# olibridge01/TeXOCR

Hardware: AMD Instinct MI355X
Metric: images/sec (OCRModel.generate, greedy, max_len=256, 224x672 px) (higher is better)
Workload: dtype bf16; 1 GPU; BASELINE configs[1]: config.yml dims (256-d/8h/4L enc + 4L dec, patch 16, PatchEmbedding C=3), batch 64/GPU, 224x672, greedy max_len=256; global_batch=64, parallelism=dp1 (images sharded, single process, no collective)

## Files before the change

### texocr_amd/csrc/common.h

```cpp
#pragma once
#include <hip/hip_runtime.h>
#include <hip/hip_bf16.h>
#include <stdint.h>

namespace txo {

typedef float f32x4 __attribute__((ext_vector_type(4)));
typedef __bf16 bf16x8 __attribute__((ext_vector_type(8)));
typedef uint32_t u32x4 __attribute__((ext_vector_type(4)));

constexpr int WAVE = 64;
constexpr float LN_EPS = 1e-5f;
constexpr float ATTN_SCALE = 0.125f;
constexpr int DH = 64;

template <typename T> struct Elem;
template <> struct Elem<float> {
    static constexpr int PER16 = 4;
    static constexpr int KCHUNK = 16;
    __device__ static inline float from_f32(float v) { return v; }
    __device__ static inline float to_f32(float v) { return v; }
};
template <> struct Elem<__hip_bfloat16> {
    static constexpr int PER16 = 8;
// ... 115 lines not shown
__device__ inline float ln_apply(float y, float mean, float rstd, float g, float b) { const float t = y - mean; return t * rstd * g + b; }

__device__ inline float gelu_erf(float x) { return 0.5f * x * (1.0f + erff(x * 0.70710678118654752440f)); }
__device__ inline float sigmoidf(float x) { return 1.0f / (1.0f + expf(-x)); }

__device__ inline float gelu_fast(float x) {
    const float z = x * 0.70710678118654752440f, a = fabsf(z);
    const float t = __builtin_amdgcn_rcpf(fmaf(0.3275911f, a, 1.0f));
    float p = fmaf(1.061405429f, t, -1.453152027f);
    p = fmaf(p, t, 1.421413741f); p = fmaf(p, t, -0.284496736f); p = fmaf(p, t, 0.254829592f);
    const float e = __builtin_amdgcn_exp2f(-a * a * 1.4426950408889634f);
    const float erf_abs = fmaf(-p * t, e, 1.0f);
    return 0.5f * x * (1.0f + copysignf(erf_abs, z));
}
__device__ inline float sigmoid_fast(float x) { return __builtin_amdgcn_rcpf(1.0f + __builtin_amdgcn_exp2f(-x * 1.4426950408889634f)); }
template <bool FAST> __device__ inline float gelu_sel(float x) { if constexpr (FAST) return gelu_fast(x); else return gelu_erf(x); }
template <bool FAST> __device__ inline float sigmoid_sel(float x) { if constexpr (FAST) return sigmoid_fast(x); else return sigmoidf(x); }

__device__ inline int swz128(int row, int piece) { return row * 128 + ((piece ^ (row & 7)) << 4); }

struct FastDiv {
    uint32_t d, m, l;
    FastDiv() : d(1), m(1), l(0) {}
    explicit FastDiv(uint32_t div) : d(div) {
        l = 0;
        while ((1u << l) < div) ++l;
        m = (uint32_t)((((uint64_t)1 << 32) * (((uint64_t)1 << l) - div)) / div + 1);
    }
    __host__ __device__ inline uint32_t div(uint32_t n) const {
#if defined(__HIP_DEVICE_COMPILE__)
        return (uint32_t)(((uint64_t)__umulhi(n, m) + n) >> l);
#else
        return (uint32_t)(((((uint64_t)n * m) >> 32) + n) >> l);
#endif
    }
    __host__ __device__ inline void divmod(uint32_t n, uint32_t& q, uint32_t& r) const { q = div(n); r = n - q * d; }
};

__device__ inline u32x4 ld16(const void* p) { return *reinterpret_cast<const u32x4*>(p); }
__device__ inline u32x4 ld16_stream(const void* p) { return __builtin_nontemporal_load(reinterpret_cast<const u32x4*>(p)); }
__device__ inline void st16(void* p, const u32x4& v) { *reinterpret_cast<u32x4*>(p) = v; }
#ifndef TXO_EXP_MALL
#define TXO_EXP_MALL 0
#endif
__device__ inline u32x4 ld16_once(const void* p) { if constexpr (TXO_EXP_MALL) return ld16_stream(p); else return ld16(p); }

__device__ inline float4 lds_ld_f4(unsigned addr) {
#if defined(__HIP_DEVICE_COMPILE__)
    return *reinterpret_cast<const __attribute__((address_space(3))) float4*>((uintptr_t)addr);
#else
    (void)addr; return float4{};
#endif
}

}
```

### texocr_amd/csrc/dec_gemm.h

```cpp
#pragma once
#include "common.h"

namespace txo {

enum { PRO_NONE = 0, PRO_EMBED = 1, PRO_LN2 = 2, PRO_LNF = 3 };
enum { EPI_QKV = 0, EPI_Q = 1, EPI_GLU_RES = 2, EPI_GEGLU = 3, EPI_BIAS_RES = 4, EPI_LOGITS = 5, EPI_STORE_T = 6 };

template <bool COH> __device__ inline float ldc_f32(const float* p) {
    if constexpr (!COH) return *p;
    else return __uint_as_float(__hip_atomic_load(reinterpret_cast<const unsigned*>(p), __ATOMIC_RELAXED, __HIP_MEMORY_SCOPE_AGENT));
}
template <bool COH> __device__ inline long long ldc_i64(const int64_t* p) {
    if constexpr (!COH) return *p;
    else return (long long)__hip_atomic_load(reinterpret_cast<const unsigned long long*>(p), __ATOMIC_RELAXED, __HIP_MEMORY_SCOPE_AGENT);
}
template <bool COH> __device__ inline u32x4 ldc16(const void* p) {
    if constexpr (!COH) return ld16(p);
    else {
        const unsigned long long* q = reinterpret_cast<const unsigned long long*>(p);
        const unsigned long long lo = __hip_atomic_load(q, __ATOMIC_RELAXED, __HIP_MEMORY_SCOPE_AGENT);
        const unsigned long long hi = __hip_atomic_load(q + 1, __ATOMIC_RELAXED, __HIP_MEMORY_SCOPE_AGENT);
        u32x4 r; r.x = (unsigned)lo; r.y = (unsigned)(lo >> 32); r.z = (unsigned)hi; r.w = (unsigned)(hi >> 32);
        return r;
    }
}
template <bool COH, typename E> __device__ inline u32x4 ldc16_at(const E* base, size_t off) {
    if constexpr (!COH) return ld16(base + off);
    else {
        const __amdgpu_buffer_rsrc_t r = __builtin_amdgcn_make_buffer_rsrc(const_cast<E*>(base), 0, 0x7fffffff, 0x00020000);
        return __builtin_amdgcn_raw_buffer_load_b128(r, (int)(off * sizeof(E)), 0, 16);
    }
}
template <bool COH> __device__ inline float4 ldc_f4_at(const float* base, size_t off) {
    const u32x4 r = ldc16_at<COH>(base, off);
    return make_float4(__uint_as_float(r.x), __uint_as_float(r.y), __uint_as_float(r.z), __uint_as_float(r.w));
}
template <bool COH> __device__ inline float4 ldc_f4(const float* p) {
    const u32x4 r = ldc16<COH>(p);
    return make_float4(__uint_as_float(r.x), __uint_as_float(r.y), __uint_as_float(r.z), __uint_as_float(r.w));
}
struct NoWait { __device__ inline void operator()() const {} };

constexpr int wfrag_regs(int KW, int BN) { return KW * (BN == 32 ? 2 : 1); }
constexpr int WBUF_REGS = 8;
struct WBuf { u32x4 r[WBUF_REGS]; };

template <typename T> struct DecGemmArgs {
    int rows, N, K;
    const T* W;
    int w_tiled;
    const float* bias;
    const T* A;
    const float* y;
    float* x_out;
    const float* gamma; const float* beta;
    unsigned ln_lds;
    const int64_t* tok; const float* tok_emb; const float* pos_emb;
    const int* t_ptr;
    int t_host;
    float* q_out;
    T* k_cache; T* v_cache;
    int inner, heads, tmax;
    const float* resid; float* y_out; int D;
    T* h_out; int F;
    T* z_cache;
    float* logits;
    unsigned long long* stamps;
    int a_tiled;
};

constexpr int DG_BM = 16, DG_BN = 32, DG_GROUP = 8;

template <int NVMAX, bool FAST>
__device__ inline void ln16(float4 (&v)[NVMAX], int nv, const float4 (&g)[NVMAX], const float4 (&b)[NVMAX], float inv_d) {
    float s = 0.f;
#pragma unroll
    for (int i = 0; i < NVMAX; ++i) if (i < nv) s += (v[i].x + v[i].y) + (v[i].z + v[i].w);
    const float mean = row16_sum(s) * inv_d;
    float q = 0.f;
#pragma unroll
    for (int i = 0; i < NVMAX; ++i) if (i < nv) {
        v[i].x -= mean; v[i].y -= mean; v[i].z -= mean; v[i].w -= mean;
        q += (v[i].x * v[i].x + v[i].y * v[i].y) + (v[i].z * v[i].z + v[i].w * v[i].w);
    }
    const float rstd = rsqrt_sel<FAST>(row16_sum(q) * inv_d + LN_EPS);
#pragma unroll
    for (int i = 0; i < NVMAX; ++i) if (i < nv) {
        v[i].x = v[i].x * rstd * g[i].x + b[i].x; v[i].y = v[i].y * rstd * g[i].y + b[i].y;
        v[i].z = v[i].z * rstd * g[i].z + b[i].z; v[i].w = v[i].w * rstd * g[i].w + b[i].w;
    }
}

template <typename T>
__device__ inline int a_off(int r, int k, int row_bytes, int pmask) {
    const int piece = (k * (int)sizeof(T)) >> 4;
    return r * row_bytes + ((piece ^ (r & pmask)) << 4) + ((k * (int)sizeof(T)) & 15);
}

template <typename T, int KW, int BN>
__device__ __forceinline__ void dec_gemm_prefetch(WBuf& f, const T* W, int N, int bx, int tid, bool real, int tiled = 0) {
    static_assert(KW > 0, "compile-time K only");
    constexpr int PER16 = Elem<T>::PER16, KCH = Elem<T>::KCHUNK, K = KW * 4 * KCH;
    static_assert(wfrag_regs(KW, BN) <= WBUF_REGS, "prefetch buffer too small");
    const int lane = tid & 63, wave = __builtin_amdgcn_readfirstlane(tid >> 6), lr = lane & 15, lg = lane >> 4;
    const int n0 = real ? bx * BN : 0;
    const T* w0 = W + (size_t)min(n0 + lr, N - 1) * K + lg * PER16;
    const T* w1 = W + (size_t)min(n0 + 16 + lr, N - 1) * K + lg * PER16;
    int wstep = KCH;
    if (tiled) {
// ... 59 lines not shown
            const int kc = wave + 4 * (g0 + c);
            fw0[c] = ld16(w0 + (size_t)kc * wstep); if constexpr (TWO) fw1[c] = ld16(w1 + (size_t)kc * wstep);
        }
    };
    auto load_a_global = [&](int g0) {
        const int m = min(m0 + lr, rows - 1);
        const bool at = !COH && a.a_tiled;
        const size_t abase = at ? ((size_t)(m >> 4) * nch * 16 + (m & 15)) * KCH : (size_t)m * K;
        const int astep = at ? 16 * KCH : KCH;
#pragma unroll
        for (int c = 0; c < GROUP; ++c) if (g0 + c < my_nch)
            fa[c] = ldc16_at<COH>(a.A, abase + (size_t)(wave + 4 * (g0 + c)) * astep + lg * PER16);
    };
    if constexpr (HASPRE) {
        static_assert(FIXED && wfrag_regs(KW, BN) <= WBUF_REGS, "prefetched fragments need a compile-time K that fits the buffer");
#pragma unroll
        for (int c = 0; c < GROUP; ++c) { fw0[c] = pre.r[c]; if constexpr (TWO) fw1[c] = pre.r[(KW + c) % WBUF_REGS]; }
    } else {
        load_w(0);
    }
    [[maybe_unused]] float4 lng[NVMAX], lnb[NVMAX];
    if constexpr (PRO != PRO_NONE) {
        const int sub = tid & 15, nv = FIXED ? NVMAX : K >> 6;
#pragma unroll
        for (int i = 0; i < NVMAX; ++i) if (i < nv) {
            if (COH && a.ln_lds) {
                lng[i] = lds_ld_f4(a.ln_lds + (i * 64 + sub * 4) * 4);
                lnb[i] = lds_ld_f4(a.ln_lds + (K + i * 64 + sub * 4) * 4);
            } else {
                lng[i] = *reinterpret_cast<const float4*>(a.gamma + i * 64 + sub * 4);
                lnb[i] = *reinterpret_cast<const float4*>(a.beta + i * 64 + sub * 4);
            }
        }
    }
    wait_prev();
    if constexpr (EPI == EPI_GLU_RES) {
        e_res0 = ldc_f32<COH>(a.resid + (size_t)emc * a.D + (n0 >> 1) + (lr & 7));
        if constexpr (TWO) e_res1 = ldc_f32<COH>(a.resid + (size_t)emc * a.D + (n0 >> 1) + 8 + (lr & 7));
    } else if constexpr (EPI == EPI_BIAS_RES) {
        e_res0 = ldc_f32<COH>(a.resid + (size_t)emc * a.D + na); e_res1 = ldc_f32<COH>(a.resid + (size_t)emc * a.D + nb);
    }
    int t = 0;
    if constexpr (PRO == PRO_EMBED || EPI == EPI_QKV || (EPI == EPI_STORE_T && PRO != PRO_NONE)) t = a.t_host >= 0 ? a.t_host : *a.t_ptr;
    if constexpr (PRO == PRO_NONE) load_a_global(0);
    __builtin_amdgcn_sched_barrier(0);

    if constexpr (PRO != PRO_NONE) {
        const int sub = tid & 15, r = tid >> 4, nv = FIXED ? NVMAX : K >> 6;
        const float inv_d = 1.0f / K;
        const int m = min(m0 + r, rows - 1);
        float4 v[NVMAX];
        float4 (&g)[NVMAX] = lng; float4 (&b)[NVMAX] = lnb;
        if constexpr (PRO == PRO_EMBED) {
            const float* te = a.tok_emb + (size_t)ldc_i64<COH>(a.tok + m) * K;
            const float* pe = a.pos_emb + (size_t)t * K;
#pragma unroll
            for (int i = 0; i < NVMAX; ++i) if (i < nv) {
                const float4 p = *reinterpret_cast<const float4*>(te + i * 64 + sub * 4);
                const float4 q = *reinterpret_cast<const float4*>(pe + i * 64 + sub * 4);
                v[i] = make_float4(p.x + q.x, p.y + q.y, p.z + q.z, p.w + q.w);
            }
        } else {
#pragma unroll
            for (int i = 0; i < NVMAX; ++i) if (i < nv)
                v[i] = ldc_f4_at<COH>(a.y, (size_t)m * K + i * 64 + sub * 4);
        }
        if constexpr (PRO == PRO_LN2) ln16<NVMAX, sizeof(T) == 2>(v, nv, g, b, inv_d);
        if constexpr (PRO == PRO_EMBED || PRO == PRO_LN2) {
            if (bx == 0 && valid && m0 + r < rows) {
#pragma unroll
                for (int i = 0; i < NVMAX; ++i) if (i < nv)
                    *reinterpret_cast<float4*>(a.x_out + (size_t)m * K + i * 64 + sub * 4) = v[i];
            }
        }
        ln16<NVMAX, sizeof(T) == 2>(v, nv, g, b, inv_d);
        [[maybe_unused]] T* zrow = nullptr;
        if constexpr (EPI == EPI_STORE_T) { if (a.z_cache && bx == 0 && valid && m0 + r < rows) zrow = a.z_cache + ((size_t)m * a.tmax + t) * K; }
#pragma unroll
        for (int i = 0; i < NVMAX; ++i) if (i < nv) {
            unsigned char* dst = smem + a_off<T>(r, i * 64 + sub * 4, row_bytes, pmask);
            if constexpr (sizeof(T) == 4) {
                *reinterpret_cast<float4*>(dst) = v[i];
                if constexpr (EPI == EPI_STORE_T) { if (zrow) *reinterpret_cast<float4*>(zrow + i * 64 + sub * 4) = v[i]; }
            } else {
                union { bf16 h[4]; uint2 u; } c;
                c.h[0] = __float2bfloat16(v[i].x); c.h[1] = __float2bfloat16(v[i].y);
                c.h[2] = __float2bfloat16(v[i].z); c.h[3] = __float2bfloat16(v[i].w);
                *reinterpret_cast<uint2*>(dst) = c.u;
                if constexpr (EPI == EPI_STORE_T) { if (zrow) *reinterpret_cast<uint2*>(zrow + i * 64 + sub * 4) = c.u; }
            }
        }
        __syncthreads();
    }

    f32x4 acc0 = {0.f, 0.f, 0.f, 0.f}, acc1 = {0.f, 0.f, 0.f, 0.f};
    for (int g0 = 0; g0 < my_nch; g0 += GROUP) {
        if (g0 > 0) { load_w(g0); if constexpr (PRO == PRO_NONE) load_a_global(g0); }
        if constexpr (PRO != PRO_NONE) {
#pragma unroll
            for (int c = 0; c < GROUP; ++c) if (g0 + c < my_nch)
                fa[c] = ld16(smem + a_off<T>(lr, (wave + 4 * (g0 + c)) * KCH + lg * PER16, row_bytes, pmask));
        }
#pragma unroll
        for (int c = 0; c < GROUP; ++c) if (g0 + c < my_nch) { mma16<T>(acc0, fa[c], fw0[c]); if constexpr (TWO) mma16<T>(acc1, fa[c], fw1[c]); }
    }

    if (a.stamps) { asm volatile("" :: "v"(acc0[0]), "v"(acc1[0])); ts1 = __builtin_amdgcn_s_memrealtime(); }
// ... 212 lines not shown
```

### texocr_amd/csrc/engine.hip

```cpp
#include "../../include/texocr.h"

#include <hip/hip_runtime.h>
#include <hip/hip_ext.h>

#include <algorithm>
#include <array>
#include <cmath>
#include <cstdio>
#include <cstdlib>
#include <chrono>
#include <cstring>
#include <map>
#include <memory>
#include <string>
#include <type_traits>
#include <vector>

namespace txo {
static thread_local std::string g_err;
static int fail(int code, const std::string& msg) { g_err = msg; return code; }
}
#define HIP_TRY(expr)                                                                                   \
    do {                                                                                                \
        hipError_t _e = (expr);                                                                         \
// ... 1710 lines not shown
        const size_t lds = persist_lds_bytes<T, D_, H_>();
        auto kern = pa.logp_out ? (sample_mode ? decode_persist_kernel<T, D_, H_, true, true> : decode_persist_kernel<T, D_, H_, false, true>)
                                : (sample_mode ? decode_persist_kernel<T, D_, H_, true, false> : decode_persist_kernel<T, D_, H_, false, false>);
        if (hipFuncSetAttribute(reinterpret_cast<const void*>(kern), hipFuncAttributeMaxDynamicSharedMemorySize, (int)lds) != hipSuccess) {
            (void)hipGetLastError();
            return fail(TXO_E_STATE, "persistent decode: the device refused the launch's dynamic LDS size");
        }
        if (prof_persist && pool.used + 2 <= pool.ev.size()) {
            hipEvent_t e0 = pool.next(), e1 = pool.next();
            hipExtLaunchKernelGGL(kern, dim3(PS_TEAMS * PS_TEAM_BLOCKS), dim3(PS_THREADS), lds, s, e0, e1, 0, pa);
            ev_persist.push_back({e0, e1});
        } else {
            hipLaunchKernelGGL(kern, dim3(PS_TEAMS * PS_TEAM_BLOCKS), dim3(PS_THREADS), lds, s, pa);
        }
        return 0;
    }
    int generate_persist(const Decode& d, int n_pos, int* n_steps, bool* broke, hipStream_t s) {
        const int B = d.src.B, N = d.src.N, eos = d.q.eos, max_len = n_pos;
        PersistArgs<T> pa{};
        pa.B = B; pa.N = N; pa.V = V; pa.Ld = cfg.dec_layers; pa.Tmax = Tmax; pa.max_len = max_len; pa.eos = eos; pa.bos = cfg.bos;
        for (int l = 0; l < cfg.dec_layers; ++l) {
            PersistLayer<T>& L = pa.L[l];
            L.wqkv = dec_self[l].wqkv; L.wo_s = dec_self[l].wo; L.bo_s = dec_self[l].bo;
            L.wq_c = dec_cross[l].wq; L.wo_c = dec_cross[l].wo; L.bo_c = dec_cross[l].bo;
            L.w1 = dec_mlp[l].w1; L.b1 = dec_mlp[l].b1; L.w2 = dec_mlp[l].w2; L.b2 = dec_mlp[l].b2;
        }
        pa.wlog = wlog;
        {
            bool all = knobs.w_tiled_on && wtiled.count(wlog);
            for (int l = 0; l < cfg.dec_layers && all; ++l)
                all = wtiled.count(dec_self[l].wqkv) && wtiled.count(dec_self[l].wo) && wtiled.count(dec_cross[l].wo) && wtiled.count(dec_mlp[l].w1) && wtiled.count(dec_mlp[l].w2);
            pa.w_tiled = all ? 1 : 0;
            if (all) {
                for (int l = 0; l < cfg.dec_layers; ++l) {
                    PersistLayer<T>& L = pa.L[l];
                    L.wqkv = wtiled.at(dec_self[l].wqkv); L.wo_s = wtiled.at(dec_self[l].wo); L.wo_c = wtiled.at(dec_cross[l].wo);
                    L.w1 = wtiled.at(dec_mlp[l].w1); L.w2 = wtiled.at(dec_mlp[l].w2);
                }
                pa.wlog = wtiled.at(wlog);
            }
        }
        pa.gamma = dec_g; pa.beta = dec_b; pa.gamma_f = decn_g; pa.beta_f = decn_b; pa.tok_emb = tok_emb; pa.pos_emb = pos_emb;
        pa.blog = blog;
        pa.dx = dx; pa.dy = dy; pa.dq = dq; pa.dlogits = dlogits; pa.dao = dao; pa.dhid = dhid;
        pa.cur_tok = cur_tok; pa.eos_seen = eos_seen; pa.skv = skv; pa.ckv = ckv;
        pa.self_stride = (size_t)ses.rows * Id * Tmax; pa.cross_stride = (size_t)ses.images * N * Id;
        pa.tokens_out = d.q.tokens; pa.out_stride = d.q.max_len; pa.logits_out = d.q.logits; pa.logp_out = d.q.logp;
        pa.sample = sample_mode; pa.sample_topk = sample_topk; pa.inv_temp = 1.0f / sample_temp; pa.seed = sample_seed;
        pa.ctl = pctl; pa.stamps = pstamps;
        const char* stamp_file = knobs.run.pstamps ? knobs.run.pstamps_file.c_str() : nullptr;
        pa.stamp_step = stamp_file ? std::min(max_len - 1, 200) : -1;
        if (knobs.run.has_stagger) pa.stagger_ticks = knobs.run.stagger_ticks;
        if (knobs.run.has_inject) pa.inject_fail = knobs.run.inject_fail;
        HIP_TRY(hipMemsetAsync(pctl, 0, sizeof(PersistCtl), s));
        if (stamp_file) HIP_TRY(hipMemsetAsync(pstamps, 0, sizeof(unsigned long long) * PS_TEAMS * PS_STAMP_RANKS * PS_MAX_STAGES * PS_STAMP_WORDS, s));
        if (D == 256) { if (int r = launch_persist<256, 8>(pa, s)) return r; }
        else if constexpr (sizeof(T) == 2) { if (int r = launch_persist<768, 12>(pa, s)) return r; }
        else return TXO_E_STATE;
        if (hipGetLastError() != hipSuccess) return fail(TXO_E_STATE, "persistent decode: the launch was refused");
        HIP_TRY(hipMemcpyAsync(pctl_host, pctl, sizeof(PersistCtl), hipMemcpyDeviceToHost, s));
        HIP_TRY(hipStreamSynchronize(s));
        const PersistCtl& c = *pctl_host;
        if (c.fail) { g_err = c.fail & 2u ? "persistent decode: a team spans more than one XCD" : "persistent decode: a hand-off timed out"; return TXO_E_STATE; }
        const int rpt = (B + PS_TEAMS - 1) / PS_TEAMS, nteams = (B + rpt - 1) / rpt;
        int steps = max_len;
        *broke = false;
        if (eos >= 0) {
            bool all = true; int last = 0;
            for (int k = 0; k < nteams; ++k) {
                const int nr = std::min(rpt, B - k * rpt);
                all = all && (int)c.eos_rows[k] >= nr;
                last = std::max(last, c.last_first_eos[k]);
            }
            if (all) steps = std::min(max_len, last + 1);
            *broke = all && last + 1 <= max_len;
        }
        for (int k = 0; k < nteams; ++k)
            if (c.steps_run[k] < steps) { g_err = "persistent decode: a team stopped before the batch's last position"; return TXO_E_STATE; }
        if (stamp_file) Stamps::dump_persist(stamp_file, pstamps, nteams, cfg.dec_layers);
        *n_steps = steps;
        return 0;
    }
    int generate_common(const Decode& d, hipStream_t s) {
        const DecodeReq& q = d.q;
        int steps = 0; last_compactions = 0;
        last_ragged = d.src.ragged();
        const int rc = generate_impl(d, &steps, s);
        ses.row_stop = false;
        ses.forced = false;
        ses.ruled = false;
        ses.closing = false;
        ses.guard_p = ses.guard_r = 0;
        rules_rows = (rules_on && rc == 0) ? d.src.B : 0;
        if (last_ragged) ses.open = false;
        if (rc) return rc;
        if (q.n_steps) *q.n_steps = steps;
        if (last_compactions > 0) ses.open = false;
        if (stop_mode == 1 && q.eos >= 0 && steps > 0 && !d.prompted()) {
            hipLaunchKernelGGL(pad_after_eos_kernel, dim3((d.src.B + 255) / 256), dim3(256), 0, s, q.tokens, q.logp, q.max_len, steps, d.src.B, q.eos, cfg.bos, cfg.pad);
            HIP_TRY(hipStreamSynchronize(s));
            HIP_TRY(hipGetLastError());
        }
        return 0;
    }
    int compact_lane(int li, int new_rows, int t1, int eos) {
        auto& ln = lanes[li];
// ... 833 lines not shown
```

### texocr_amd/csrc/persist.h

```cpp
#pragma once
#include "dec_attn.h"
#include "dec_gemm.h"
#include "step.h"

#ifndef TXO_PS_ATTN_STAMPS
#define TXO_PS_ATTN_STAMPS false
#endif

namespace txo {

constexpr bool PS_ATTN_STAMPS = TXO_PS_ATTN_STAMPS;
constexpr int PS_TEAMS = 8, PS_TEAM_BLOCKS = 32, PS_THREADS = 512, PS_MAXLD = 8;
constexpr int PS_MAX_STAGES = 7 * PS_MAXLD + 2, PS_STAMP_RANKS = 4, PS_STAMP_WORDS = 8;

struct PersistCtl {
    unsigned flags[PS_TEAMS][32];
    unsigned xcc_mask[PS_TEAMS];
    unsigned eos_rows[PS_TEAMS];
    int last_first_eos[PS_TEAMS];
    unsigned stop[PS_TEAMS];
    int steps_run[PS_TEAMS];
    unsigned done_mask;
    unsigned fail;
    unsigned pad[2];
};
static_assert(sizeof(PersistCtl) % 16 == 0, "memset block");

template <typename T> struct PersistLayer {
    const T* wqkv; const T* wo_s; const float* bo_s;
    const T* wq_c; const T* wo_c; const float* bo_c;
    const T* w1; const float* b1; const T* w2; const float* b2;
};

template <typename T> struct PersistArgs {
    int B, N, V, Ld, Tmax, max_len, eos, bos;
    PersistLayer<T> L[PS_MAXLD];
    const float *gamma, *beta, *gamma_f, *beta_f, *tok_emb, *pos_emb, *blog;
    const T* wlog;
    float *dx, *dy, *dq, *dlogits; T *dao, *dhid;
    int64_t* cur_tok; int* eos_seen;
    T *skv, *ckv; size_t self_stride, cross_stride;
    int64_t* tokens_out; int out_stride; float* logits_out;
    float* logp_out;
    PersistCtl* ctl;
    int w_tiled;
    int sample; int sample_topk; float inv_temp; unsigned long long seed;
    int inject_fail;
    int stagger_ticks;
    unsigned long long* stamps; int stamp_step;
};

typedef unsigned u32x8 __attribute__((ext_vector_type(8)));
__device__ inline unsigned min8(const u32x8& v) {
    return min(min(min(v[0], v[1]), min(v[2], v[3])), min(min(v[4], v[5]), min(v[6], v[7])));
}
constexpr unsigned PS_GIVE_UP_TICKS = 400000u;
constexpr unsigned PS_GIVE_UP_FIRST_TICKS = 2000000u;

struct TeamSync {
    unsigned* flags;
    int rank; unsigned epoch;
    unsigned* fail; int* lds_dead; bool armed, dead;
    unsigned long long* stp;
    __device__ inline void operator()() {
        if (!armed) return;
// ... 9 lines not shown
                             "s_load_dwordx8 %0, %5, 0x0\n\t"
                             "s_load_dwordx8 %1, %5, 0x20\n\t"
                             "s_load_dwordx8 %2, %5, 0x40\n\t"
                             "s_load_dwordx8 %3, %5, 0x60\n\t"
                             "s_load_dword %4, %6, 0x0\n\t"
                             "s_waitcnt lgkmcnt(0)"
                             : "=&s"(f0), "=&s"(f1), "=&s"(f2), "=&s"(f3), "=&s"(fl) : "s"(flags), "s"(fail) : "memory");
                const unsigned behind = min(min(min8(f0), min8(f1)), min(min8(f2), min8(f3)));
                if (behind >= epoch) break;
                if (fl != 0u || ((++spins & 63u) == 0u && __builtin_amdgcn_s_memrealtime() - t_begin > (epoch <= 2u ? PS_GIVE_UP_FIRST_TICKS : PS_GIVE_UP_TICKS))) {
                    if (lane == 0) { atomicOr(fail, 1u); *lds_dead = 1; }
                    break;
                }
                __builtin_amdgcn_s_sleep(1);
            }
            if (stp && threadIdx.x == 0) stp[1] = __builtin_amdgcn_s_memrealtime();
        }
        __syncthreads();
        dead = dead || *lds_dead != 0;
    }
    __device__ inline void arrive() {
        if (stp && threadIdx.x == 0) stp[2] = __builtin_amdgcn_s_memrealtime();
        asm volatile("s_waitcnt vmcnt(0)" ::: "memory");
        __syncthreads();
        ++epoch;
        if (threadIdx.x == 0) {
            if (stp) stp[3] = __builtin_amdgcn_s_memrealtime();
            __hip_atomic_store(flags + rank, epoch, __ATOMIC_RELAXED, __HIP_MEMORY_SCOPE_WORKGROUP);
            if (stp) { asm volatile("s_waitcnt vmcnt(0)" ::: "memory"); stp[4] = __builtin_amdgcn_s_memrealtime(); stp += PS_STAMP_WORDS; }
        }
        armed = true;
    }
};

template <typename T> constexpr int ps_kw_pro(int K) { const int kw = K / (4 * Elem<T>::KCHUNK); return (kw == 2 || kw == 4 || kw == 6) ? kw : 0; }
template <typename T> constexpr int ps_kw_half(int K) {
    const int kw = K / (4 * Elem<T>::KCHUNK); return (kw == 4 || kw == 6 || kw == 8 || kw == 12 || kw == 16) ? kw : 0;
}

template <typename T, int D_, int HEADS_>
constexpr size_t persist_group_lds() {
    size_t g = (size_t)DG_BM * D_ * sizeof(T) + 8192;
    if (g < sizeof(DecAttnLds<false>)) g = sizeof(DecAttnLds<false>);
    return (g + 255) & ~(size_t)255;
}

template <typename T, int D_>
constexpr bool persist_w2_in_lds() {
    return sizeof(T) == 2 && ps_kw_half<T>(4 * D_) > 0 && wfrag_regs(ps_kw_half<T>(4 * D_), 16) <= WBUF_REGS && D_ / 16 == 16;
}
template <typename T, int D_, int HEADS_>
constexpr size_t persist_lds_bytes() {
    return 2 * persist_group_lds<T, D_, HEADS_>() + 16 + (persist_w2_in_lds<T, D_>() ? 2 * (size_t)WBUF_REGS * 256 * 16 : 0) +
           4 * (size_t)D_ * sizeof(float);
}

template <typename T, int D_, int HEADS_, bool SAMPLE, bool LOGP>
__global__ __launch_bounds__(PS_THREADS) void decode_persist_kernel(PersistArgs<T> a) {
    constexpr int D = D_, HEADS = HEADS_, ID = HEADS * DH, F = 4 * D;
    constexpr size_t GLDS = persist_group_lds<T, D_, HEADS_>();
    extern __shared__ __attribute__((aligned(16))) unsigned char smem_all[];
    const int team = blockIdx.x % PS_TEAMS, rank = blockIdx.x / PS_TEAMS;
    const int grp = __builtin_amdgcn_readfirstlane(threadIdx.x >> 8);
    int tid = threadIdx.x & 255;
    unsigned char* smem = smem_all + (size_t)grp * GLDS;
    int* lds_dead = reinterpret_cast<int*>(smem_all + 2 * GLDS);
    const int sa = grp * PS_TEAM_BLOCKS + rank;
    constexpr int NSB = PS_TEAM_BLOCKS * 2;

    const int rpt = (a.B + PS_TEAMS - 1) / PS_TEAMS;
    const int r0 = team * rpt, nr = max(0, min(a.B - r0, rpt));
    if (nr == 0) return;
    const int nteams = (a.B + rpt - 1) / rpt;
    const unsigned full_mask = (1u << nteams) - 1u;
    const int nrt = (nr + DG_BM - 1) / DG_BM;

    PersistCtl* ctl = a.ctl;
    if (threadIdx.x == 0) {
        *lds_dead = 0;
        unsigned id;
        asm volatile("s_getreg_b32 %0, hwreg(HW_REG_XCC_ID)" : "=s"(id));
        atomicOr(&ctl->xcc_mask[team], 1u << (id & 15u));
        if (rank == 0 && a.eos >= 0 && a.bos == a.eos) {
            __hip_atomic_store(&ctl->eos_rows[team], (unsigned)nr, __ATOMIC_RELAXED, __HIP_MEMORY_SCOPE_AGENT);
        }
    }
    if (a.stagger_ticks > 0 && team > 0) {
        const unsigned long long t0 = __builtin_amdgcn_s_memrealtime(), until = (unsigned long long)a.stagger_ticks * team;
        while (__builtin_amdgcn_s_memrealtime() - t0 < until) __builtin_amdgcn_s_sleep(8);
    }
    __syncthreads();
    TeamSync ts{&ctl->flags[team][0], rank, 0u, &ctl->fail, lds_dead, false, false, nullptr};
    bool placement_checked = false;

    float* ln_lds = reinterpret_cast<float*>(smem_all + 2 * GLDS + 16 + (persist_w2_in_lds<T, D_>() ? 2 * (size_t)WBUF_REGS * 256 * 16 : 0));
    for (int c = threadIdx.x; c < D; c += PS_THREADS) {
        ln_lds[c] = a.gamma[c]; ln_lds[D + c] = a.beta[c]; ln_lds[2 * D + c] = a.gamma_f[c]; ln_lds[3 * D + c] = a.beta_f[c];
    }
    __syncthreads();
    const unsigned ln_lds_addr = (unsigned)(uintptr_t)ln_lds;

    DecGemmArgs<T> gb{};
    gb.ln_lds = ln_lds_addr; gb.w_tiled = a.w_tiled;
    gb.rows = nr; gb.gamma = a.gamma; gb.beta = a.beta; gb.t_ptr = nullptr; gb.D = D; gb.inner = ID; gb.heads = HEADS; gb.tmax = a.Tmax;
    float* lx = a.dx + (size_t)r0 * D; float* ly = a.dy + (size_t)r0 * D; float* lq = a.dq + (size_t)r0 * ID;
    T* lao = a.dao + (size_t)r0 * ID; T* lhid = a.dhid + (size_t)r0 * F; float* llog = a.dlogits + (size_t)r0 * a.V;
    const int srank = rank == 0 ? 0 : (rank == 10 ? 1 : (rank == 20 ? 2 : (rank == PS_TEAM_BLOCKS - 1 ? 3 : -1)));
    unsigned long long* stamp_base = (a.stamps && srank >= 0 && threadIdx.x == 0)
        ? a.stamps + ((size_t)team * PS_STAMP_RANKS + srank) * PS_MAX_STAGES * PS_STAMP_WORDS : nullptr;

    constexpr int KWP = ps_kw_pro<T>(D), KWI = ps_kw_half<T>(ID), KWF = ps_kw_half<T>(F);
    constexpr int NC_QKV = (3 * ID + 31) / 32, NC_O = 2 * D / 16, NC_F1 = 2 * F / 32, NC_F2 = D / 16;
    const int nc_log = (a.V + 31) / 32;

    constexpr bool W2_LDS_OK = persist_w2_in_lds<T, D_>();
    const bool w2_lds = W2_LDS_OK && a.Ld <= PS_TEAM_BLOCKS / 8;
    const int w2_layer = (rank >> 4) + 2 * grp, w2_tile = rank & 15;
    unsigned char* w2_lds_base = smem_all + 2 * GLDS + 16 + (size_t)grp * (WBUF_REGS * 256 * 16);
    if constexpr (W2_LDS_OK) {
        if (w2_lds && w2_layer < a.Ld) {
            WBuf park;
            dec_gemm_prefetch<T, KWF, 16>(park, a.L[w2_layer].w2, D, w2_tile, tid, true, a.w_tiled);
#pragma unroll
            for (int c = 0; c < KWF; ++c) st16(w2_lds_base + ((size_t)c * 256 + tid) * 16, park.r[c]);
        }
    }

    int t = 0;
    for (; t < a.max_len; ++t) {
        asm volatile("" : "+v"(tid));
        gb.t_host = t;
        if (a.inject_fail > 0 && t == a.inject_fail && team == 0 && rank == 0) {
            if (threadIdx.x == 0) { atomicOr(&ctl->fail, 1u); *lds_dead = 1; }
            __syncthreads();
            ts.dead = true;
            break;
        }
        int stage = 0;
        ts.stp = (stamp_base && t == a.stamp_step) ? stamp_base : nullptr;
#define PS_GEMM(PRO, EPI, KW, BN, ARGS, NCOL)                                                                           \
        do {                                                                                                            \
            const int ncol_ = (NCOL), nt_ = ncol_ * nrt;                                                                \
            for (int base_ = 0; base_ < nt_; base_ += NSB) {                                                            \
                if (base_ > 0) __syncthreads();                            \
                if (base_ + rank < nt_) {                                   \
                    const int tile_ = base_ + sa;                                                                       \
                    if (tile_ >= nt_) dec_gemm_idle<PRO>(ts);                                                           \
                    else if (base_ == 0) {                                                                              \
                        auto args_ = ARGS;                                                                              \
                        args_.stamps = (ts.stp && grp == 0) ? ts.stp + 5 - 3 * tile_ : nullptr;    \
                        dec_gemm_tile<T, PRO, EPI, KW, BN, true>(args_, tile_ % ncol_, tile_ / ncol_, tid, smem, true, ts); \
                    }                                                                                                   \
                    else dec_gemm_tile<T, PRO, EPI, KW, BN, true>(ARGS, tile_ % ncol_, tile_ / ncol_, tid, smem, true, ts); \
                } else if (base_ == 0) ts();                                                                            \
            }                                                                                                           \
            ts();                                                                                                       \
            ts.arrive();                                                                                                \
            ++stage;                                                                                                    \
        } while (0)
#define PS_ATTN(MODE, APRO, NLV, ARGS, LK)                                                                              \
        do {                                                                                                            \
            const int np_ = nr * HEADS;                                                                                 \
            for (int base_ = 0; base_ < np_; base_ += NSB) {                                                            \
                if (base_ > 0) __syncthreads();                                                                         \
                if (base_ + rank < np_) {                                                                               \
                    const int p_ = base_ + sa;                                                                          \
                    if (p_ >= np_) dec_attn_idle<T, MODE, APRO, NLV>((LK), ts);                                         \
                    else if (base_ == 0) {                                                                              \
                        auto args_ = ARGS;                                                                              \
                        args_.stamps = (PS_ATTN_STAMPS && ts.stp && grp == 0) ? ts.stp + 5 - 3 * p_ : nullptr;    \
                        dec_attn_tile<T, MODE, APRO, NLV, 1, false, false, true>(args_, p_, tid,                       \
                            *reinterpret_cast<DecAttnLds<false>*>(smem), true, ts); \
                    }                                                                                                   \
                    else dec_attn_tile<T, MODE, APRO, NLV, 1, false, false, true>(ARGS, p_, tid,          \
                        *reinterpret_cast<DecAttnLds<false>*>(smem), true, ts); \
                } else if (base_ == 0) ts();                                                                            \
            }                                                                                                           \
            ts();                                                                                                       \
            ts.arrive();                                                                                                \
            ++stage;                                                                                                    \
        } while (0)
        for (int l = 0; l < a.Ld; ++l) {
            asm volatile("" : "+v"(tid));
            const PersistLayer<T>& W = a.L[l];
            T* kc = a.skv + (size_t)(2 * l) * a.self_stride + (size_t)r0 * HEADS * a.Tmax * DH;
            T* vc = a.skv + (size_t)(2 * l + 1) * a.self_stride + (size_t)r0 * HEADS * a.Tmax * DH;
            {
                DecGemmArgs<T> g = gb; g.N = 3 * ID; g.K = D; g.W = W.wqkv; g.y = ly; g.x_out = lx;
                g.tok = a.cur_tok + r0; g.tok_emb = a.tok_emb; g.pos_emb = a.pos_emb; g.q_out = lq; g.k_cache = kc; g.v_cache = vc;
                if (l == 0) PS_GEMM(PRO_EMBED, EPI_QKV, KWP, 32, g, NC_QKV);
                else PS_GEMM(PRO_LN2, EPI_QKV, KWP, 32, g, NC_QKV);
            }
            if (!placement_checked) {
                placement_checked = true;
                ts();
                if (threadIdx.x == 0) {
                    const unsigned m = __hip_atomic_load(&ctl->xcc_mask[team], __ATOMIC_RELAXED, __HIP_MEMORY_SCOPE_AGENT);
                    if (__builtin_popcount(m) != 1) { atomicOr(&ctl->fail, 2u); *lds_dead = 1; }
                }
                __syncthreads();
                ts.dead = ts.dead || *lds_dead != 0;
            }
            if (ts.dead) break;
            DecAttnArgs<T> at{};
            at.gamma = a.gamma; at.beta = a.beta; at.D = D; at.heads = HEADS; at.t_host = t; at.kv_div = 1; at.path = nullptr;
            at.y = ly; at.x_out = lx; at.out = lao; at.qin = lq; at.tok = a.cur_tok + r0; at.tok_emb = a.tok_emb; at.pos_emb = a.pos_emb;
            {
                DecAttnArgs<T> s = at; s.W = W.wqkv; s.K = kc; s.V = vc; s.lmax = a.Tmax; s.len = 0;
                PS_ATTN(ATT_SELF, APRO_NONE, (sizeof(T) == 2 ? 8 : 16), s, t + 1);
            }
            {
                DecGemmArgs<T> g = gb; g.N = 2 * D; g.K = ID; g.W = W.wo_s; g.bias = W.bo_s; g.A = lao; g.resid = lx; g.y_out = ly;
                PS_GEMM(PRO_NONE, EPI_GLU_RES, KWI, 16, g, NC_O);
            }
            if (ts.dead) break;
            {
                DecAttnArgs<T> s = at; s.W = W.wq_c;
                s.K = a.ckv + (size_t)(2 * l) * a.cross_stride + (size_t)r0 * HEADS * a.N * DH;
                s.V = a.ckv + (size_t)(2 * l + 1) * a.cross_stride + (size_t)r0 * HEADS * a.N * DH;
                s.lmax = a.N; s.len = a.N;
                PS_ATTN(ATT_CROSS, APRO_LN2, DA_NL_CROSS, s, a.N);
            }
            {
                DecGemmArgs<T> g = gb; g.N = 2 * D; g.K = ID; g.W = W.wo_c; g.bias = W.bo_c; g.A = lao; g.resid = lx; g.y_out = ly;
                PS_GEMM(PRO_NONE, EPI_GLU_RES, KWI, 16, g, NC_O);
            }
            if (ts.dead) break;
            {
                DecGemmArgs<T> g = gb; g.N = 2 * F; g.K = D; g.W = W.w1; g.bias = W.b1; g.y = ly; g.x_out = lx; g.h_out = lhid; g.F = F;
                PS_GEMM(PRO_LN2, EPI_GEGLU, KWP, 32, g, NC_F1);
                DecGemmArgs<T> h = gb; h.N = D; h.K = F; h.W = W.w2; h.bias = W.b2; h.A = lhid; h.resid = lx; h.y_out = ly;
                bool w2_done = false;
                if constexpr (W2_LDS_OK) {
                    if (w2_lds) {
                        w2_done = true;
                        if ((rank >> 4) != (l & 1)) {
                            ts();
                        } else if (w2_layer != l) {
                            for (int by = 0; by < nrt; ++by) {
                                if (by > 0) __syncthreads();
                                dec_gemm_idle<PRO_NONE>(ts);
                            }
                        } else {
                            WBuf wb;
#pragma unroll
                            for (int c = 0; c < KWF; ++c) wb.r[c] = ld16(w2_lds_base + ((size_t)c * 256 + tid) * 16);
                            for (int by = 0; by < nrt; ++by) {
                                if (by > 0) __syncthreads();
                                auto args_ = h;
                                args_.stamps = (ts.stp && by == 0) ? ts.stp + 5 - 3 * w2_tile : nullptr;
                                dec_gemm_tile_pre<T, PRO_NONE, EPI_BIAS_RES, KWF, 16, true, true>(args_, w2_tile, by, tid, smem, true, ts, wb);
                            }
                        }
                        ts();
                        ts.arrive();
                        ++stage;
                    }
                }
                if (!w2_done) PS_GEMM(PRO_NONE, EPI_BIAS_RES, KWF, 16, h, NC_F2);
            }
            if (ts.dead) break;
        }
        if (ts.dead) break;
        {
            DecGemmArgs<T> g = gb; g.N = a.V; g.K = D; g.W = a.wlog; g.bias = a.blog; g.logits = llog; g.y = ly;
            g.gamma = a.gamma_f; g.beta = a.beta_f; g.ln_lds = ln_lds_addr + 2 * D * (unsigned)sizeof(float);
            PS_GEMM(PRO_LNF, EPI_LOGITS, KWP, 32, g, nc_log);
        }
        {
            ts();
            const int lane = threadIdx.x & 63;
            for (int r = (int)(threadIdx.x >> 6) * PS_TEAM_BLOCKS + rank; r < nr && !ts.dead; r += PS_TEAM_BLOCKS * (PS_THREADS / 64)) {
                const int row = r0 + r;
                const float* lg = a.dlogits + (size_t)row * a.V;
                float* lo = a.logits_out ? a.logits_out + ((size_t)row * a.out_stride + t) * a.V : nullptr;
                float best = -3.4e38f; int bi = 0x7fffffff;
                constexpr bool lp = LOGP;
                [[maybe_unused]] float logp = 0.f, lm = -3.4e38f, ls = 0.f;
                if constexpr (SAMPLE) {
                    auto ld = [&](int j) { return ldc_f32<true>(lg + j); };
                    auto ld4 = [&](int j) { return ldc16_at<true>(a.dlogits, (size_t)row * a.V + j); };
                    bi = sample_row_regs(ld, ld4, lo, a.V, lane, a.sample_topk, a.inv_temp, a.seed, (unsigned)row, (unsigned)t, lp, logp);
                } else {
                if ((a.V & 3) == 0) {
                    const int n4 = a.V >> 2;
                    for (int base = 0; base < n4; base += 256) {
                        float4 v[4];
#pragma unroll
                        for (int u = 0; u < 4; ++u) {
                            const int j4 = base + u * 64 + lane;
                            v[u] = ldc_f4_at<true>(a.dlogits, (size_t)row * a.V + (size_t)min(j4, n4 - 1) * 4);
                        }
#pragma unroll
                        for (int u = 0; u < 4; ++u) {
                            const int j4 = base + u * 64 + lane;
                            if (j4 >= n4) continue;
                            if (lo) reinterpret_cast<float4*>(lo)[j4] = v[u];
                            if constexpr (lp) lse_push4(lm, ls, v[u]);
                            const int j = j4 * 4;
                            if (v[u].x > best) { best = v[u].x; bi = j; }
                            if (v[u].y > best) { best = v[u].y; bi = j + 1; }
                            if (v[u].z > best) { best = v[u].z; bi = j + 2; }
                            if (v[u].w > best) { best = v[u].w; bi = j + 3; }
                        }
                    }
                } else {
                    for (int j = lane; j < a.V; j += 64) {
                        const float v = ldc_f32<true>(lg + j);
                        if (lo) lo[j] = v;
                        if constexpr (lp) lse_push(lm, ls, v);
                        if (v > best) { best = v; bi = j; }
                    }
                }
                wave_argmax(best, bi);
                if constexpr (lp) logp = -lse_finish(lm, ls, best);
                }
                if (lane == 0) {
                    bi = in_vocab(bi, a.V);
                    a.cur_tok[row] = bi;
                    a.tokens_out[(size_t)row * a.out_stride + t] = bi;
                    if constexpr (lp) a.logp_out[(size_t)row * a.out_stride + t] = logp;
                    if (a.eos >= 0 && bi == a.eos &&
                        __hip_atomic_load(reinterpret_cast<unsigned*>(a.eos_seen + row), __ATOMIC_RELAXED, __HIP_MEMORY_SCOPE_AGENT) == 0u) {
                        __hip_atomic_store(reinterpret_cast<unsigned*>(a.eos_seen + row), 1u, __ATOMIC_RELAXED, __HIP_MEMORY_SCOPE_AGENT);
                        const int prev_max = atomicMax(&ctl->last_first_eos[team], t);
                        asm volatile("s_waitcnt vmcnt(0)" :: "v"(prev_max) : "memory");
                        __hip_atomic_fetch_add(&ctl->eos_rows[team], 1u, __ATOMIC_RELAXED, __HIP_MEMORY_SCOPE_AGENT);
                    }
                }
            }
            if (a.eos >= 0 && rank == 0 && threadIdx.x == 0) {
                const unsigned n = __hip_atomic_load(&ctl->eos_rows[team], __ATOMIC_RELAXED, __HIP_MEMORY_SCOPE_AGENT);
                if (n >= (unsigned)nr) {
                    const unsigned bit = 1u << team;
                    const unsigned old = atomicOr(&ctl->done_mask, bit);
                    if (((old | bit) & full_mask) == full_mask) {
                        int need = 0;
                        for (int k = 0; k < nteams; ++k) need = max(need, atomicMax(&ctl->last_first_eos[k], 0));
                        if (t >= need) __hip_atomic_store(&ctl->stop[team], 1u, __ATOMIC_RELAXED, __HIP_MEMORY_SCOPE_AGENT);
                    }
                }
            }
            ts.arrive();
            ++stage;
        }
        ts();
        if (ts.dead) break;
        if (a.eos >= 0 && __hip_atomic_load(&ctl->stop[team], __ATOMIC_RELAXED, __HIP_MEMORY_SCOPE_AGENT)) { ++t; break; }
    }
#undef PS_GEMM
#undef PS_ATTN
    if (rank == 0 && threadIdx.x == 0) ctl->steps_run[team] = t;
}

}
```

### texocr_amd/csrc/stamps.h

```cpp
#pragma once
#include "persist.h"

namespace txo {

struct Stamps {
    static constexpr int BLOCKS = 2048, KERNELS = 64;
    unsigned long long* buf = nullptr; int slot = -1;
    std::vector<std::string> names;
    unsigned long long* next(const char* name) {
        if (slot < 0 || slot >= KERNELS) return nullptr;
        names.push_back(name);
        return buf + (size_t)(slot++) * BLOCKS * 3;
    }
    int begin(hipStream_t s) { HIP_TRY(hipMemsetAsync(buf, 0, sizeof(unsigned long long) * KERNELS * BLOCKS * 3, s)); slot = 0; names.clear(); return 0; }
    void dump(const char* file, const std::string* raw, hipStream_t s) {
        const int nk = slot; slot = -1;
        std::vector<unsigned long long> h((size_t)nk * BLOCKS * 3);
        if (hipStreamSynchronize(s) != hipSuccess) return;
        if (hipMemcpy(h.data(), buf, h.size() * sizeof(unsigned long long), hipMemcpyDeviceToHost) != hipSuccess) return;
        FILE* f = fopen(file, "w");
        if (!f) return;
        unsigned long long t0 = ~0ull;
        for (auto v : h) if (v && v < t0) t0 = v;
        for (int k2 = 0; k2 < nk; ++k2) {
            unsigned long long first = ~0ull, last_in = 0, mid_lo = ~0ull, mid_hi = 0, first_out = ~0ull, last = 0; int nb = 0;
            for (int b = 0; b < BLOCKS; ++b) {
                const unsigned long long* d = &h[((size_t)k2 * BLOCKS + b) * 3];
                if (!d[0]) continue;
                ++nb; first = std::min(first, d[0]); last_in = std::max(last_in, d[0]); mid_lo = std::min(mid_lo, d[1]); mid_hi = std::max(mid_hi, d[1]);
                first_out = std::min(first_out, d[2]); last = std::max(last, d[2]);
            }
            fprintf(f, "%-24s blocks %4d | first entry %7.2f us, last entry %7.2f | operands/panel done %7.2f .. %7.2f | first exit %7.2f, last exit %7.2f\n",
                    names[k2].c_str(), nb, (first - t0) / 100.0, (last_in - t0) / 100.0, (mid_lo - t0) / 100.0, (mid_hi - t0) / 100.0,
                    (first_out - t0) / 100.0, (last - t0) / 100.0);
        }
        if (raw) {
            for (int k2 = 0; k2 < nk; ++k2) {
                if (names[k2].find(*raw) == std::string::npos) continue;
                for (int b = 0; b < BLOCKS; ++b) {
                    const unsigned long long* d = &h[((size_t)k2 * BLOCKS + b) * 3];
                    if (d[0]) fprintf(f, "raw %d %-24s block %4d  %7.2f %7.2f %7.2f\n", k2, names[k2].c_str(), b, (d[0] - t0) / 100.0, (d[1] - t0) / 100.0, (d[2] - t0) / 100.0);
                }
            }
        }
        fclose(f);
    }
    static void dump_persist(const char* file, const unsigned long long* dev, int nteams, int layers) {
        const int ns = 7 * layers + 2;
        std::vector<unsigned long long> h((size_t)PS_TEAMS * PS_STAMP_RANKS * PS_MAX_STAGES * PS_STAMP_WORDS);
        if (hipMemcpy(h.data(), dev, h.size() * sizeof(unsigned long long), hipMemcpyDeviceToHost) != hipSuccess) return;
        FILE* f = fopen(file, "w");
        if (!f) return;
        static const char* names[7] = {"LN+qkv gemm", "self attention", "self out-proj+GLU+res", "cross attention (LN+q fused)",
                                       "cross out-proj+GLU+res", "LN+ffn-in+GeGLU", "ffn-out+res"};
        static const int ranks[PS_STAMP_RANKS] = {0, 10, 20, PS_TEAM_BLOCKS - 1};
        fprintf(f, "# persistent decode launch, ONE decode position, workgroups of rank 0 / 10 / 20 / 31 of every team.  Per stage, us:\n"
                   "#   poll  = polling the team counter for the previous stage's arrivals (weights / K panel already requested)\n"
                   "#   work  = barrier + read the previous stage's rows (sc1) + compute + issue the stores\n"
                   "#   drain = s_waitcnt vmcnt(0) of every wave + workgroup barrier\n"
                   "#   pub   = the arrival atomic, issued -> returned\n"
                   "#   end   = time of publication since the position's first stamp\n");
        for (int k = 0; k < nteams; ++k)
            for (int r = 0; r < PS_STAMP_RANKS; ++r) {
                const unsigned long long* d = &h[((size_t)k * PS_STAMP_RANKS + r) * PS_MAX_STAGES * PS_STAMP_WORDS];
                if (!d[2]) continue;
                const unsigned long long t0 = d[2];
                fprintf(f, "team %d rank %d: position span %.2f us\n", k, ranks[r], (d[(ns - 1) * PS_STAMP_WORDS + 4] - t0) / 100.0);
                if (k > 1) continue;
                for (int i = 0; i < ns; ++i) {
                    const unsigned long long* e = d + i * PS_STAMP_WORDS;
                    const char* nm = i < 7 * layers ? names[i % 7] : (i == 7 * layers ? "LNf+logits" : "argmax+append");
                    fprintf(f, "  L%-2d %-30s poll %5.2f  work %5.2f  drain %5.2f  pub %5.2f | end %7.2f", i < 7 * layers ? i / 7 : -1, nm,
                            e[0] ? (e[1] - e[0]) / 100.0 : 0.0, e[1] ? (e[2] - e[1]) / 100.0 : 0.0, (e[3] - e[2]) / 100.0, (e[4] - e[3]) / 100.0,
                            (e[4] - t0) / 100.0);
                    const bool attn = i < 7 * layers && (i % 7 == 1 || i % 7 == 3);
                    if (e[5] && e[1] && !attn)
                        fprintf(f, " | tile: seen->mfma done %5.2f  reduce %5.2f  epilogue+stores %5.2f", (e[6] - e[1]) / 100.0, (e[7] - e[6]) / 100.0, (e[2] - e[7]) / 100.0);
                    if (e[5] && e[1] && attn)
                        fprintf(f, " | tile: seen->panel consumed %5.2f  reduce+store %5.2f  (other group / barrier %5.2f)", ((long long)e[6] - (long long)e[1]) / 100.0,
                                (e[7] - e[6]) / 100.0, ((long long)e[2] - (long long)e[7]) / 100.0);
                    if (e[5] && e[0] && i > 0)
                        fprintf(f, " | pre: setup %5.2f  requests %5.2f", ((long long)e[5] - (long long)(e - PS_STAMP_WORDS)[4]) / 100.0, ((long long)e[0] - (long long)e[5]) / 100.0);
                    fprintf(f, "\n");
                }
            }
        fclose(f);
    }
};

}
```

Measured before the change: 2009 images/sec.

## Replicate greedy argmax in every workgroup to drop the token hand-off barrier

Every workgroup in a team now runs the argmax over all of its team's rows itself and keeps the chosen tokens in a small LDS array. The next position's embedding prologue reads tokens from that LDS copy, so the team-wide arrival and poll after the argmax stage goes away. Only rank 0 writes tokens, logp and EOS bookkeeping to global memory, and the EOS stop check moves into layer 0 after self-attention. The cost is redundant argmax work over the vocabulary in every workgroup, plus a new cap on rows per team.

```diff
diff --git a/texocr_amd/csrc/common.h b/texocr_amd/csrc/common.h
--- a/texocr_amd/csrc/common.h
+++ b/texocr_amd/csrc/common.h
@@ -191,5 +191,12 @@
     (void)addr; return float4{};
 #endif
 }
-
-}
+__device__ inline int lds_ld_i32(unsigned addr) {
+#if defined(__HIP_DEVICE_COMPILE__)
+    return *reinterpret_cast<const __attribute__((address_space(3))) int*>((uintptr_t)addr);
+#else
+    (void)addr; return 0;
+#endif
+}
+
+}
diff --git a/texocr_amd/csrc/dec_gemm.h b/texocr_amd/csrc/dec_gemm.h
--- a/texocr_amd/csrc/dec_gemm.h
+++ b/texocr_amd/csrc/dec_gemm.h
@@ -55,6 +55,7 @@
     float* x_out;
     const float* gamma; const float* beta;
     unsigned ln_lds;
+    unsigned tok_lds;
     const int64_t* tok; const float* tok_emb; const float* pos_emb;
     const int* t_ptr;
     int t_host;
@@ -220,7 +221,8 @@
         float4 v[NVMAX];
         float4 (&g)[NVMAX] = lng; float4 (&b)[NVMAX] = lnb;
         if constexpr (PRO == PRO_EMBED) {
-            const float* te = a.tok_emb + (size_t)ldc_i64<COH>(a.tok + m) * K;
+            const long long tk = (COH && a.tok_lds) ? (long long)lds_ld_i32(a.tok_lds + m * 4) : ldc_i64<COH>(a.tok + m);
+            const float* te = a.tok_emb + (size_t)tk * K;
             const float* pe = a.pos_emb + (size_t)t * K;
 #pragma unroll
             for (int i = 0; i < NVMAX; ++i) if (i < nv) {
diff --git a/texocr_amd/csrc/engine.hip b/texocr_amd/csrc/engine.hip
--- a/texocr_amd/csrc/engine.hip
+++ b/texocr_amd/csrc/engine.hip
@@ -1786,6 +1786,7 @@
         pa.stamp_step = stamp_file ? std::min(max_len - 1, 200) : -1;
         if (knobs.run.has_stagger) pa.stagger_ticks = knobs.run.stagger_ticks;
         if (knobs.run.has_inject) pa.inject_fail = knobs.run.inject_fail;
+        if ((B + PS_TEAMS - 1) / PS_TEAMS > PS_TEAM_ROWS_MAX) return fail(TXO_E_STATE, "persistent decode: more rows per team than its token copy holds");
         HIP_TRY(hipMemsetAsync(pctl, 0, sizeof(PersistCtl), s));
         if (stamp_file) HIP_TRY(hipMemsetAsync(pstamps, 0, sizeof(unsigned long long) * PS_TEAMS * PS_STAMP_RANKS * PS_MAX_STAGES * PS_STAMP_WORDS, s));
         if (D == 256) { if (int r = launch_persist<256, 8>(pa, s)) return r; }
diff --git a/texocr_amd/csrc/persist.h b/texocr_amd/csrc/persist.h
--- a/texocr_amd/csrc/persist.h
+++ b/texocr_amd/csrc/persist.h
@@ -11,6 +11,7 @@
 
 constexpr bool PS_ATTN_STAMPS = TXO_PS_ATTN_STAMPS;
 constexpr int PS_TEAMS = 8, PS_TEAM_BLOCKS = 32, PS_THREADS = 512, PS_MAXLD = 8;
+constexpr int PS_TEAM_ROWS_MAX = 128;
 constexpr int PS_MAX_STAGES = 7 * PS_MAXLD + 2, PS_STAMP_RANKS = 4, PS_STAMP_WORDS = 8;
 
 struct PersistCtl {
@@ -126,7 +127,8 @@
 template <typename T, int D_, int HEADS_>
 constexpr size_t persist_lds_bytes() {
     return 2 * persist_group_lds<T, D_, HEADS_>() + 16 + (persist_w2_in_lds<T, D_>() ? 2 * (size_t)WBUF_REGS * 256 * 16 : 0) +
-           4 * (size_t)D_ * sizeof(float);
+           4 * (size_t)D_ * sizeof(float) +
+           PS_TEAM_ROWS_MAX * sizeof(int);
 }
 
 template <typename T, int D_, int HEADS_, bool SAMPLE, bool LOGP>
@@ -171,11 +173,13 @@
     for (int c = threadIdx.x; c < D; c += PS_THREADS) {
         ln_lds[c] = a.gamma[c]; ln_lds[D + c] = a.beta[c]; ln_lds[2 * D + c] = a.gamma_f[c]; ln_lds[3 * D + c] = a.beta_f[c];
     }
+    int* tok_lds = reinterpret_cast<int*>(ln_lds + 4 * D);
+    if ((int)threadIdx.x < min(nr, PS_TEAM_ROWS_MAX)) tok_lds[threadIdx.x] = (int)a.cur_tok[r0 + threadIdx.x];
     __syncthreads();
     const unsigned ln_lds_addr = (unsigned)(uintptr_t)ln_lds;
 
     DecGemmArgs<T> gb{};
-    gb.ln_lds = ln_lds_addr; gb.w_tiled = a.w_tiled;
+    gb.ln_lds = ln_lds_addr; gb.tok_lds = ln_lds_addr + 4 * D * (unsigned)sizeof(float); gb.w_tiled = a.w_tiled;
     gb.rows = nr; gb.gamma = a.gamma; gb.beta = a.beta; gb.t_ptr = nullptr; gb.D = D; gb.inner = ID; gb.heads = HEADS; gb.tmax = a.Tmax;
     float* lx = a.dx + (size_t)r0 * D; float* ly = a.dy + (size_t)r0 * D; float* lq = a.dq + (size_t)r0 * ID;
     T* lao = a.dao + (size_t)r0 * ID; T* lhid = a.dhid + (size_t)r0 * F; float* llog = a.dlogits + (size_t)r0 * a.V;
@@ -261,7 +265,7 @@
             T* vc = a.skv + (size_t)(2 * l + 1) * a.self_stride + (size_t)r0 * HEADS * a.Tmax * DH;
             {
                 DecGemmArgs<T> g = gb; g.N = 3 * ID; g.K = D; g.W = W.wqkv; g.y = ly; g.x_out = lx;
-                g.tok = a.cur_tok + r0; g.tok_emb = a.tok_emb; g.pos_emb = a.pos_emb; g.q_out = lq; g.k_cache = kc; g.v_cache = vc;
+                g.tok_emb = a.tok_emb; g.pos_emb = a.pos_emb; g.q_out = lq; g.k_cache = kc; g.v_cache = vc;
                 if (l == 0) PS_GEMM(PRO_EMBED, EPI_QKV, KWP, 32, g, NC_QKV);
                 else PS_GEMM(PRO_LN2, EPI_QKV, KWP, 32, g, NC_QKV);
             }
@@ -278,11 +282,12 @@
             if (ts.dead) break;
             DecAttnArgs<T> at{};
             at.gamma = a.gamma; at.beta = a.beta; at.D = D; at.heads = HEADS; at.t_host = t; at.kv_div = 1; at.path = nullptr;
-            at.y = ly; at.x_out = lx; at.out = lao; at.qin = lq; at.tok = a.cur_tok + r0; at.tok_emb = a.tok_emb; at.pos_emb = a.pos_emb;
+            at.y = ly; at.x_out = lx; at.out = lao; at.qin = lq;
             {
                 DecAttnArgs<T> s = at; s.W = W.wqkv; s.K = kc; s.V = vc; s.lmax = a.Tmax; s.len = 0;
                 PS_ATTN(ATT_SELF, APRO_NONE, (sizeof(T) == 2 ? 8 : 16), s, t + 1);
             }
+            if (l == 0 && t > 0 && a.eos >= 0 && __hip_atomic_load(&ctl->stop[team], __ATOMIC_RELAXED, __HIP_MEMORY_SCOPE_AGENT)) { ts.dead = true; break; }
             {
                 DecGemmArgs<T> g = gb; g.N = 2 * D; g.K = ID; g.W = W.wo_s; g.bias = W.bo_s; g.A = lao; g.resid = lx; g.y_out = ly;
                 PS_GEMM(PRO_NONE, EPI_GLU_RES, KWI, 16, g, NC_O);
@@ -344,10 +349,11 @@
         {
             ts();
             const int lane = threadIdx.x & 63;
-            for (int r = (int)(threadIdx.x >> 6) * PS_TEAM_BLOCKS + rank; r < nr && !ts.dead; r += PS_TEAM_BLOCKS * (PS_THREADS / 64)) {
+            const bool side = rank == 0;
+            for (int r = (int)(threadIdx.x >> 6); r < nr && !ts.dead; r += PS_THREADS / 64) {
                 const int row = r0 + r;
                 const float* lg = a.dlogits + (size_t)row * a.V;
-                float* lo = a.logits_out ? a.logits_out + ((size_t)row * a.out_stride + t) * a.V : nullptr;
+                float* lo = (side && a.logits_out) ? a.logits_out + ((size_t)row * a.out_stride + t) * a.V : nullptr;
                 float best = -3.4e38f; int bi = 0x7fffffff;
                 constexpr bool lp = LOGP;
                 [[maybe_unused]] float logp = 0.f, lm = -3.4e38f, ls = 0.f;
@@ -391,15 +397,18 @@
                 }
                 if (lane == 0) {
                     bi = in_vocab(bi, a.V);
-                    a.cur_tok[row] = bi;
-                    a.tokens_out[(size_t)row * a.out_stride + t] = bi;
-                    if constexpr (lp) a.logp_out[(size_t)row * a.out_stride + t] = logp;
-                    if (a.eos >= 0 && bi == a.eos &&
-                        __hip_atomic_load(reinterpret_cast<unsigned*>(a.eos_seen + row), __ATOMIC_RELAXED, __HIP_MEMORY_SCOPE_AGENT) == 0u) {
-                        __hip_atomic_store(reinterpret_cast<unsigned*>(a.eos_seen + row), 1u, __ATOMIC_RELAXED, __HIP_MEMORY_SCOPE_AGENT);
-                        const int prev_max = atomicMax(&ctl->last_first_eos[team], t);
-                        asm volatile("s_waitcnt vmcnt(0)" :: "v"(prev_max) : "memory");
-                        __hip_atomic_fetch_add(&ctl->eos_rows[team], 1u, __ATOMIC_RELAXED, __HIP_MEMORY_SCOPE_AGENT);
+                    tok_lds[r] = bi;
+                    if (side) {
+                        a.cur_tok[row] = bi;
+                        a.tokens_out[(size_t)row * a.out_stride + t] = bi;
+                        if constexpr (lp) a.logp_out[(size_t)row * a.out_stride + t] = logp;
+                        if (a.eos >= 0 && bi == a.eos &&
+                            __hip_atomic_load(reinterpret_cast<unsigned*>(a.eos_seen + row), __ATOMIC_RELAXED, __HIP_MEMORY_SCOPE_AGENT) == 0u) {
+                            __hip_atomic_store(reinterpret_cast<unsigned*>(a.eos_seen + row), 1u, __ATOMIC_RELAXED, __HIP_MEMORY_SCOPE_AGENT);
+                            const int prev_max = atomicMax(&ctl->last_first_eos[team], t);
+                            asm volatile("s_waitcnt vmcnt(0)" :: "v"(prev_max) : "memory");
+                            __hip_atomic_fetch_add(&ctl->eos_rows[team], 1u, __ATOMIC_RELAXED, __HIP_MEMORY_SCOPE_AGENT);
+                        }
                     }
                 }
             }
@@ -415,12 +424,10 @@
                     }
                 }
             }
-            ts.arrive();
-            ++stage;
-        }
-        ts();
+            __syncthreads();
+            if (ts.stp && threadIdx.x == 0) ts.stp[2] = __builtin_amdgcn_s_memrealtime();
+        }
         if (ts.dead) break;
-        if (a.eos >= 0 && __hip_atomic_load(&ctl->stop[team], __ATOMIC_RELAXED, __HIP_MEMORY_SCOPE_AGENT)) { ++t; break; }
     }
 #undef PS_GEMM
 #undef PS_ATTN
diff --git a/texocr_amd/csrc/stamps.h b/texocr_amd/csrc/stamps.h
--- a/texocr_amd/csrc/stamps.h
+++ b/texocr_amd/csrc/stamps.h
@@ -46,7 +46,7 @@
         fclose(f);
     }
     static void dump_persist(const char* file, const unsigned long long* dev, int nteams, int layers) {
-        const int ns = 7 * layers + 2;
+        const int ns = 7 * layers + 1;
         std::vector<unsigned long long> h((size_t)PS_TEAMS * PS_STAMP_RANKS * PS_MAX_STAGES * PS_STAMP_WORDS);
         if (hipMemcpy(h.data(), dev, h.size() * sizeof(unsigned long long), hipMemcpyDeviceToHost) != hipSuccess) return;
         FILE* f = fopen(file, "w");
@@ -59,17 +59,19 @@
                    "#   work  = barrier + read the previous stage's rows (sc1) + compute + issue the stores\n"
                    "#   drain = s_waitcnt vmcnt(0) of every wave + workgroup barrier\n"
                    "#   pub   = the arrival atomic, issued -> returned\n"
-                   "#   end   = time of publication since the position's first stamp\n");
+                   "#   end   = time of publication since the position's first stamp\n"
+                   "# local pick (no hand-off): poll = the wait for the logits, pick = this workgroup picks all of its team's rows (rank 0 also\n"
+                   "#   writes them out) up to the barrier behind which the next position starts\n");
         for (int k = 0; k < nteams; ++k)
             for (int r = 0; r < PS_STAMP_RANKS; ++r) {
                 const unsigned long long* d = &h[((size_t)k * PS_STAMP_RANKS + r) * PS_MAX_STAGES * PS_STAMP_WORDS];
                 if (!d[2]) continue;
                 const unsigned long long t0 = d[2];
-                fprintf(f, "team %d rank %d: position span %.2f us\n", k, ranks[r], (d[(ns - 1) * PS_STAMP_WORDS + 4] - t0) / 100.0);
+                fprintf(f, "team %d rank %d: position span %.2f us\n", k, ranks[r], (d[ns * PS_STAMP_WORDS + 2] - t0) / 100.0);
                 if (k > 1) continue;
                 for (int i = 0; i < ns; ++i) {
                     const unsigned long long* e = d + i * PS_STAMP_WORDS;
-                    const char* nm = i < 7 * layers ? names[i % 7] : (i == 7 * layers ? "LNf+logits" : "argmax+append");
+                    const char* nm = i < 7 * layers ? names[i % 7] : "LNf+logits";
                     fprintf(f, "  L%-2d %-30s poll %5.2f  work %5.2f  drain %5.2f  pub %5.2f | end %7.2f", i < 7 * layers ? i / 7 : -1, nm,
                             e[0] ? (e[1] - e[0]) / 100.0 : 0.0, e[1] ? (e[2] - e[1]) / 100.0 : 0.0, (e[3] - e[2]) / 100.0, (e[4] - e[3]) / 100.0,
                             (e[4] - t0) / 100.0);
@@ -83,6 +85,8 @@
                         fprintf(f, " | pre: setup %5.2f  requests %5.2f", ((long long)e[5] - (long long)(e - PS_STAMP_WORDS)[4]) / 100.0, ((long long)e[0] - (long long)e[5]) / 100.0);
                     fprintf(f, "\n");
                 }
+                const unsigned long long* e = d + ns * PS_STAMP_WORDS;
+                fprintf(f, "  L-1 %-30s poll %5.2f  pick %5.2f | end %7.2f\n", "local pick (every workgroup)", (e[1] - e[0]) / 100.0, (e[2] - e[1]) / 100.0, (e[2] - t0) / 100.0);
             }
         fclose(f);
     }
```

New measurement: 2023 images/sec (median of 4 runs). Within noise of the previous version (+0.7%).
